# ArchDD/CPP-Raytracer-Rasterizer

Hardware: AMD Instinct MI355X
Metric: Mrays/s (primary+shadow) (higher is better)
Workload: dtype f32

## Files before the change

cpp-raytracer-rasterizer_amd/capi/binned.cpp:

```cpp
#include "capi.hpp"

namespace mirt {


int PairList::ensure(size_t cap)
{
    int r;
    if ((r = dev_realloc(&d_entries, cap)) || (r = dev_realloc(&d_pair_keys, cap)) || (r = dev_realloc(&d_pair_vals, cap)) ||
        (r = dev_realloc(&d_sorted_keys, cap)) || (r = dev_realloc(&d_tmp_vals, cap))) { cap_entries = 0; return r; }
    cap_entries = (uint32_t)cap;
    return MIRT_OK;
}


void PairList::poll()
{
    if (count_pending && hipEventQuery(ev_count) == hipSuccess) {
        known_pairs = *h_count; have_known = true; count_pending = false;
    }
    (void)hipGetLastError();
}

int PairList::record_count()
{
// ... 211 lines not shown
int transient_light_pass(LightPass &L, const float *origins, int nlights, int cube_bins, int tshells, uint32_t per_light, uint64_t lkey, bool *kept,
                         unsigned long long *zero_hits )
{
    int rc;
    const uint64_t key = Fnv(g.scene_version).mix(&lkey, 8).mix(&cube_bins, 4).mix(&tshells, 4).mix(&g.n, 4).mix(&nlights, 4).h;
    const PassPlan plan = L.kept.plan_for(key, nlights, L.pairs);
    *kept = plan.reuse;
    if (plan.reuse) return MIRT_OK;
    if ((rc = ensure_face_lists(L, nlights))) return rc;
    if (nlights > L.light_tab_lights || L.light_tab_n != g.n) {
        if ((rc = dev_grow(&L.d_light_tab, &L.light_tab_lights, nlights, (size_t)nlights * g.n, true))) return rc;
        L.light_tab_n = g.n;
    }
    const uint32_t nkeys = per_light * (uint32_t)nlights;
    if (nkeys + 1 > L.cap_bins && (rc = dev_grow(&L.d_bin_off, &L.cap_bins, nkeys + 1, (size_t)nkeys + 1, true))) return rc;
    if (!L.d_frames) HIP_TRY(hipMalloc(reinterpret_cast<void **>(&L.d_frames), sizeof(BinFrameDesc) * (6 * MIRT_MAX_LIGHTS) + sizeof(float) * 3 * (1 + MIRT_MAX_LIGHTS)));
    struct { BinFrameDesc frames[6 * MIRT_MAX_LIGHTS]; float origins[3 * (1 + MIRT_MAX_LIGHTS)]; } up;
    static_assert(sizeof(BinFrameDesc) % 4 == 0, "descriptors are uploaded as words");
    fill_light_frames(up.frames, origins, nlights, cube_bins, tshells, 0u, g.bbox_lo, g.bbox_hi);
    float *d_origins = reinterpret_cast<float *>(L.d_frames + 6 * nlights);
    memcpy(reinterpret_cast<char *>(up.frames + 6 * nlights), origins, sizeof(float) * 3 * (1 + nlights));
    const ZeroJob zj = { L.d_bin_counters, (int)(LIGHT_COUNTER_BYTES / 4), reinterpret_cast<uint32_t *>(zero_hits), zero_hits ? 2 * HIT_SHARDS * HIT_SHARD_STRIDE : 0 };
    HIP_TRY(upload_small(L.d_frames, &up, sizeof(BinFrameDesc) * 6 * nlights + sizeof(float) * 3 * (1 + nlights), g.stream, &zj));
    if ((rc = cube_bin_chain(L, L.d_frames, d_origins, nlights, nkeys, L.d_light_tab, L.d_bin_off, L.d_bin_counters, &L.kept.bin_entries, plan.may_guess))) return rc;
    L.kept.keep(key, nlights);
    if (L.cap_light_rows < L.pairs.cap_entries && (rc = dev_grow(&L.d_light_rows, &L.cap_light_rows, L.pairs.cap_entries, (size_t)L.pairs.cap_entries, true))) return rc;
    const uint32_t expect = std::max<uint32_t>(L.kept.bin_entries, 1u);
    hipLaunchKernelGGL(k_expand_light_rows, dim3((unsigned)std::min<uint32_t>((expect + 255) / 256, 4096u)), dim3(256), 0, g.stream,
                       L.d_bin_off, L.pairs.d_entries, nlights, per_light, L.d_light_tab, g.n, L.d_light_rows, L.d_bin_counters, L.pairs.cap_used, (uint32_t *)nullptr);
    return MIRT_OK;
}


int OriginTables::ensure_cam_rows() { return cam_tab_n == g.n ? MIRT_OK : dev_grow(&d_cam_tab, &cam_tab_n, g.n, (size_t)g.n, false); }

int BinPass::ensure_counters(size_t bytes)
{
    if (!d_bin_counters) { HIP_TRY(hipMalloc(reinterpret_cast<void **>(&d_bin_counters), bytes)); HIP_TRY(hipMemsetAsync(d_bin_counters, 0, bytes, g.stream)); }
    return MIRT_OK;
}

int CameraPass::ensure_sel()
{
    if (sel_n == g.n) return MIRT_OK;
    kept.forget();
    return dev_grow(&d_sel, &sel_n, g.n, (size_t)g.n, true);
}

SelectOut CameraPass::select_out(const OriginTables &T, int count_word) const
{
    SelectOut so;
    memset(&so, 0, sizeof so);
    so.cam_tab = T.d_cam_tab; so.sel = d_sel;
    so.sel_count = d_bin_counters + count_word; so.sel_count_next = d_bin_counters + (count_word ^ 1);
    return so;
}

static void launch_prep_select(const BinFrameDesc &frame, const SelectOut &so)
{
    const unsigned sel_grid = (unsigned)std::min<long long>(((long long)g.n + 1023) / 1024, (long long)g.cu_count);
    if (sel_grid) hipLaunchKernelGGL(k_prep_select, dim3(sel_grid), dim3(1024), 0, g.stream, g.d_tris, g.n, frame, so);
}

int binned_pass(const mirt_view *view, StreamState &ss, const float *origins, int nlights, int y0, int y1, BinnedPass *bp)
{
    int rc;
    CameraPass &S = ss.cam;
// ... 46 lines not shown
    if (!S.d_frames) HIP_TRY(hipMalloc(reinterpret_cast<void **>(&S.d_frames), sizeof(BinFrameDesc) * (1 + 6 * MIRT_MAX_LIGHTS)));
    const PassPlan plan = S.kept.plan_for(key, bin_mode, S.pairs);
    const uint32_t pairs_x = (uint32_t)((bs.frame0.nbu + 1) / 2);
    uint32_t group_rows[ORDER_GROUPS] = { 0 };
    for (int j = bs.frame0.j0; j < bs.frame0.j1; j++) group_rows[((uint32_t)j >> ORDER_STRIPE_SHIFT) & (ORDER_GROUPS - 1)]++;
    const uint32_t order_seg = pairs_x * *std::max_element(group_rows, group_rows + ORDER_GROUPS);
    const uint32_t *cam_off = S.d_bin_off - (size_t)key_shift_tiles * (size_t)bs.frame0.nshell;
    bool lights_kept = false, forked = false;
    if (transient) {
        static const bool side_off = env_int("MIRT_LIGHT_SIDE_STREAM", 1) == 0;
        hipStream_t main_stream = g.stream;
        forked = !plan.reuse && !side_off;
        if (forked) {
            HIP_TRY(hipEventRecord(ss.ev_fork, main_stream));
            HIP_TRY(hipStreamWaitEvent(ss.aux, ss.ev_fork, 0));
            g.stream = ss.aux;
        }
        rc = transient_light_pass(L, origins, nlights, cube_bins, tshells, per_light, lkey, &lights_kept, plan.reuse ? g.d_hits : nullptr);
        g.stream = main_stream;
        if (rc) return rc;
        if (forked) HIP_TRY(hipEventRecord(ss.ev_join, ss.aux));
    }
    if (plan.reuse) {
        if (!(transient && !lights_kept)) HIP_TRY(hipMemsetAsync(g.d_hits, 0, HIT_BYTES, g.stream));
        g.stats.bins_reused = 1;
    } else {
        S.sel_parity ^= 1;
        SelectOut so = S.select_out(ss.tabs, SEL_COUNT0 + S.sel_parity);
        so.zero_hits = g.d_hits; so.zero_counter = S.d_bin_counters;
        if ((rc = hist_prepare(ss.hist, bs.frame0, &so))) return rc;
        launch_prep_select(bs.frame0, so);
        if ((rc = hist_publish(ss.hist))) return rc;
        bs.sel = S.d_sel; bs.sel_count = so.sel_count;
        g.stats_sel_count = so.sel_count;
        if ((rc = bin_pass(S.pairs, bs, ss.tabs.d_cam_tab, nullptr, S.d_bin_counters, S.d_bin_off, &S.kept.bin_entries, plan.may_guess))) return rc;
        S.kept.keep(key, bin_mode);
        if (order_seg > S.cap_order && (rc = dev_grow(&S.d_order, &S.cap_order, order_seg, (size_t)ORDER_GROUPS * ORDER_CLASSES * order_seg, true))) return rc;
        hipLaunchKernelGGL(k_tile_order, dim3((pairs_x + 63) / 64, (unsigned)(bs.frame0.j1 - bs.frame0.j0)), dim3(64), 0, g.stream, cam_off, bs.frame0.nshell,
                           bs.frame0.nbu, bs.frame0.j0, bs.frame0.j1, S.d_bin_counters, S.pairs.cap_used, S.d_order, order_seg);
    }
    if (forked) HIP_TRY(hipStreamWaitEvent(g.stream, ss.ev_join, 0));
    k_end(MIRT_K_BIN);

    bp->cam_off = cam_off;
    bp->tiles_x = bs.frame0.nbu;
    bp->cam_shells = bs.frame0.nshell;
    bp->shell_d0 = bs.frame0.shell_d0; bp->shell_iw = bs.frame0.shell_iw;
    bp->order_seg = order_seg;
    bp->cube = transient ? cube_view(L, cube_bins, tshells) : cube_view(g.lc);
    bp->light_tab = transient ? L.d_light_tab : g.lc.d_light_tab;
    bp->light_pair_count = transient ? L.d_bin_counters : S.d_bin_counters;
    bp->light_pair_cap = transient ? L.pairs.cap_used : 0xFFFFFFFFu;
    return MIRT_OK;
}

int hist_only_pass(const mirt_view *view)
{
    int rc;
    g.stream = g.cur().stream;
    StreamState &ss = g.cur();
    CameraPass &S = ss.cam;
    if ((rc = ss.tabs.ensure_cam_rows()) || (rc = S.ensure_sel()) || (rc = S.ensure_counters(512))) return rc;
    S.kept.forget();
    const BinFrameDesc fr = make_camera_frame(view, 0, 0, g.aa);
    SelectOut so = S.select_out(ss.tabs, HIST_SEL_COUNT);
    if ((rc = hist_prepare(ss.hist, fr, &so))) return rc;
// ... 62 lines not shown
```

cpp-raytracer-rasterizer_amd/capi/capi.hpp:

```cpp
#pragma once

#include "../csrc/bin_sort.hpp"
#include "../csrc/comm.hpp"
#include "../csrc/cull.hpp"
#include "../csrc/dof.hpp"
#include "../csrc/rt_common.hpp"
#include "../csrc/raster_common.hpp"
#include "../csrc/rt_binned.hpp"
#include "../csrc/rt_trace_frame.hpp"
#include "../csrc/scan.hpp"
#include "../query/rt_query.hpp"
#include "../along/along.hpp"
#include "../along/alongs.hpp"
#include "../grid/ray_grid.hpp"
#include "../order/ordered_hits.hpp"
#include "../lights/many_lights.hpp"
#include "../lights/aa_many_lights.hpp"
#include "cube_plan.hpp"
#include "pass_plan.hpp"
#include "along_plan.hpp"
#include "object_plan.hpp"
#include "dof_plan.hpp"
#include "aa_plan.hpp"
#include "env.hpp"
// ... 30 lines not shown
MIRT_KERNEL void k_tile_order(const uint32_t *, int, int, int, int, uint32_t *, uint32_t, TilePairRec *, uint32_t);
MIRT_KERNEL void k_geo_table(const float *, int, GeoRow *, ShadeRow *);
MIRT_KERNEL void k_expand_light_rows(const uint32_t *, const uint32_t *, int, uint32_t, const OriginRow *, int, LightRow *, const uint32_t *, uint32_t, uint32_t *);
MIRT_KERNEL void k_cull(const float *, int, const CullParams, uint8_t *);
size_t rt_trace_lds_bytes(int waves);
int launch_raster(RasterFrame &f, RasterScratch &s, uint64_t scene_version, hipStream_t stream, hipEvent_t *ev, bool *ev_used);

extern char g_err[512];
int fail(int code, const char *fmt, ...);

#define HIP_TRY(expr)                                                                          \
    do {                                                                                       \
        hipError_t e_ = (expr);                                                                \
        if (e_ != hipSuccess)                                                                  \
            return fail(MIRT_ERR_HIP, "%s failed: %s (%s:%d)", #expr, hipGetErrorString(e_), __FILE__, __LINE__); \
    } while (0)

enum { EV_CALL0 = 0, EV_CALL1 = 1, EV_K0 = 2, EV_COUNT = 2 + 2 * 8 };
constexpr int MAX_FLIGHT = 4;
constexpr int SEL_COUNT0 = 80;
constexpr int HIST_SEL_COUNT = 82;
constexpr int HIST_RING = 4;
constexpr int HIST_SLOTS = HIST_RING + 1;
constexpr size_t HIT_BYTES = sizeof(unsigned long long) * HIT_SHARDS * HIT_SHARD_STRIDE;

struct OriginTables {
    OriginRow *d_cam_tab = nullptr;
    OriginRow *d_light_tab = nullptr;
    int cam_tab_n = 0, light_tab_n = 0, light_tab_lights = 0;
    float *d_origins = nullptr;
    uint32_t *d_flags = nullptr;

    int ensure_cam_rows();
    void release();
};

struct PairList {
    uint32_t *d_entries = nullptr;
    uint32_t *d_pair_keys = nullptr, *d_pair_vals = nullptr, *d_sorted_keys = nullptr;
    uint32_t *d_tmp_vals = nullptr;
    uint32_t *d_bucket = nullptr;
    uint32_t cap_buckets = 0;
    bool bucket_dirty = false;
    uint32_t cap_entries = 0;
    uint32_t cap_used = 0;
    uint32_t *h_count = nullptr;
    hipEvent_t ev_count = nullptr;
    bool count_pending = false;
    bool count_event_due = false;
    bool have_known = false;
    uint32_t known_pairs = 0;

    int ensure(size_t cap);
    void poll();
    int record_count();
    void forget_scene() { have_known = false; count_pending = false; }
    void release();
};

struct KeptPass {
    uint64_t bin_key = 0;
    bool bin_key_valid = false;
    int last_bin_mode = -1;
    uint32_t bin_entries = 0;

    PassPlan plan_for(uint64_t key, int mode, PairList &P) const;
// ... 595 lines not shown
```

cpp-raytracer-rasterizer_amd/csrc/rt_binned.hip:

```cpp
#include "rt_binned.hpp"

#include <float.h>

namespace mirt {

constexpr int BIN_L0 = BIN_COARSE * BIN_COARSE;

struct BinItem {
    float A0[4], A1[4], A2[4], Bu[4], Bv[4];
    float lou, hiu, lov, hiv;
};

__device__ __forceinline__ float bcastf(float v, int lane) { return __builtin_bit_cast(float, __builtin_amdgcn_readlane(__builtin_bit_cast(int, v), lane)); }

__device__ __forceinline__ float corner(float s, float lo, float hi) { return fmaxf(s * lo, s * hi); }

__device__ __forceinline__ bool cell_may_hit(const BinItem &u, const float (&A)[4], float I, float J, float K)
{
    bool ok = true;
#pragma unroll
    for (int k = 0; k < 4; k++) ok = ok && (__builtin_fmaf(J, u.Bv[k], __builtin_fmaf(I, u.Bu[k], A[k])) >= 0.0f);
    return ok && (I + K >= u.lou) && (I <= u.hiu) && (J + K >= u.lov) && (J <= u.hiv);
}

// ... 325 lines not shown
        if (from_cam_list) { chunk = w; frame = 0; list = bs.sel; nhere = nsel; }
        else if (faces_listed) {
            const uint32_t w2 = (uint32_t)(w - ncam);
            int lo = 0, hi = nrest;
            while (hi - lo > 1) { const int mid = (lo + hi) >> 1; if (s_first[mid] <= w2) lo = mid; else hi = mid; }
            chunk = (int)(w2 - s_first[lo]);
            frame = lo + (listed ? 1 : 0);
            list = bs.face_lists + (size_t)lo * bs.face_stride;
            nhere = min(bs.face_counts[lo], (uint32_t)n);
        } else { const int w2 = w - ncam; chunk = w2 / nrest; frame = w2 - chunk * nrest + (listed ? 1 : 0); }
        const int item_tris = from_cam_list ? cam_chunk : chunk_tris;
        const uint32_t slot = (uint32_t)chunk * (uint32_t)item_tris + threadIdx.x;
        const uint32_t tri = ((int)threadIdx.x < item_tris && slot < nhere) ? (list ? list[slot] : slot) : 0xFFFFFFFFu;
        const BinFrameDesc fr = bs.frames ? bs.frames[frame] : bs.frame0;
        BinFrameGrid gr;
        gr.nbu = fr.nbu; gr.fj0 = fr.j0; gr.fj1 = fr.j1; gr.fbase = fr.base; gr.nshell = (uint32_t)max(fr.nshell, 1);
        gr.cells_x = (gr.nbu + BIN_L0 - 1) / BIN_L0; gr.cy0 = gr.fj0 / BIN_L0;
        gr.ncell = gr.cells_x * ((gr.fj1 + BIN_L0 - 1) / BIN_L0 - gr.cy0);
        const int nbu = gr.nbu, fj0 = gr.fj0, fj1 = gr.fj1;
        BinItem it;
        memset(&it, 0, sizeof it);
        int kind = 0;
#ifdef MIRT_BIN_STATS
        int dbg_state = 0;
        bool dbg_joint = false;
#endif
        int i_lo = 0, i_hi = -1, j_lo = 0, j_hi = -1;
        unsigned long long cells = 0;
        uint32_t shell = 0;
        if (tri < (uint32_t)n && fj1 > fj0) {
            const OriginRow &row = (fr.tab == 0) ? cam_tab[tri] : light_tab[(size_t)(fr.tab - 1) * n + tri];
            shell = bin_shell_of(row.r1.w, fr.shell_d0, fr.shell_iw, fr.nshell);
            TriBinFns t = make_bin_fns(row, fr);
            add_bbox(t, tris15 + (size_t)15 * tri, fr);
#ifdef MIRT_BIN_STATS
            dbg_state = t.bstate == BOX_VALID ? 0 : (t.bstate == BOX_NONE ? 1 : 2);
#endif
            const float T = 1.6940658945086007e-21f;
            const bool both = fabsf(t.nb) < T || !(t.nb == t.nb);
            const float sgn = t.nb < 0.0f ? -1.0f : 1.0f;
            const EdgeFn *fn[4] = { &t.n, &t.p, &t.q, &t.s };
            const float inf = __builtin_huge_valf();
#pragma unroll
            for (int k = 0; k < 4; k++) {
                const float su = sgn * fn[k]->cu, sv = sgn * fn[k]->cv;
                const float base = sgn * fn[k]->c0 + fn[k]->m + su * fr.ulo + sv * fr.vlo;
                it.Bu[k] = both ? 0.0f : su * fr.du;
                it.Bv[k] = both ? 0.0f : sv * fr.dv;
                it.A0[k] = both ? inf : base + corner(su, fr.pad_lo, (float)BIN_L0 * fr.du + fr.pad_hi) + corner(sv, fr.pad_lo, (float)BIN_L0 * fr.dv + fr.pad_hi);
                it.A1[k] = both ? inf : base + corner(su, fr.pad_lo, (float)BIN_COARSE * fr.du + fr.pad_hi) + corner(sv, fr.pad_lo, (float)BIN_COARSE * fr.dv + fr.pad_hi);
                it.A2[k] = both ? inf : base + corner(su, fr.pad_lo, fr.du + fr.pad_hi) + corner(sv, fr.pad_lo, fr.dv + fr.pad_hi);
            }
            if (t.bstate == BOX_VALID) {
                box_to_bins(t.bu0, t.bu1, fr.ulo, fr.pad_lo, fr.pad_hi, bin_rcp(fr.du), &it.lou, &it.hiu);
                box_to_bins(t.bv0, t.bv1, fr.vlo, fr.pad_lo, fr.pad_hi, bin_rcp(fr.dv), &it.lov, &it.hiv);
            } else if (t.bstate == BOX_EMPTY) {
                it.lou = it.lov = inf; it.hiu = it.hiv = -inf;
            } else {
                it.lou = it.lov = -inf; it.hiu = it.hiv = inf;
            }
            const float flo_u = fmaxf(ceilf(it.lou) - 1.0f, 0.0f), fhi_u = fminf(floorf(it.hiu), (float)(nbu - 1));
            const float flo_v = fmaxf(ceilf(it.lov) - 1.0f, (float)fj0), fhi_v = fminf(floorf(it.hiv), (float)(fj1 - 1));
            if (flo_u <= fhi_u && flo_v <= fhi_v) {
                i_lo = (int)flo_u; i_hi = (int)fhi_u; j_lo = (int)flo_v; j_hi = (int)fhi_v;
                kind = (i_hi - i_lo < BIN_DIRECT_SIDE && j_hi - j_lo < BIN_DIRECT_SIDE) ? 1 : 2;
            }
// ... 163 lines not shown
```

cpp-raytracer-rasterizer_amd/csrc/rt_binned.hpp:

```cpp
#pragma once

#include "rt_common.hpp"

namespace mirt {

#ifndef MIRT_ORDER_STRIPE_SHIFT
#define MIRT_ORDER_STRIPE_SHIFT 2
#endif
constexpr int ORDER_STRIPE_SHIFT = MIRT_ORDER_STRIPE_SHIFT;
constexpr int BIN_TILE = 8;
constexpr int BIN_COARSE = 8;
constexpr int CUBE_BINS_MIN = 64;
constexpr int MAX_BIN_FRAMES = 1 + 6 * MIRT_MAX_LIGHTS;

struct BinFrameDesc {
    float P0[3], Pu[3], Pv[3];
    float S[3];
    float ru[3], rv[3], rw[3];
    float ulo, vlo, du, dv;
    float pad_lo, pad_hi;
    float dmax;
    int nbu, nbv;
    int j0, j1;
    uint32_t base;
// ... 6 lines not shown
{
    if (nshell <= 1) return 0u;
    const float s = (near - d0) * iw;
#ifdef __HIP_DEVICE_COMPILE__
    return (uint32_t)min(max((int)s, 0), nshell - 1);
#else
    if (!(s >= 0.0f)) return 0u;
    return s >= (float)(nshell - 1) ? (uint32_t)(nshell - 1) : (uint32_t)(int)s;
#endif
}

struct GeoRow { float4 g0, g1, g2; };
struct ShadeRow { float4 n, col; };
typedef OriginRow LightRow;

struct BinSet {
    const BinFrameDesc *frames;
    BinFrameDesc frame0;
    int nframes;
    uint32_t nbins;
    uint32_t *bin_off;
    uint32_t *entries;
    uint32_t cap_entries;
    uint32_t *counters;
    uint32_t *bucket_cnt;
    uint32_t nbuckets;
    int bucket_shift;
    int chunk_tris;
    const uint32_t *sel;
    const uint32_t *sel_count;
    const uint32_t *face_lists;
    const uint32_t *face_counts;
    uint32_t face_stride;
};

constexpr int SEL_HIST_MAX = 256;
struct SelectOut {
    OriginRow *cam_tab;
    uint32_t *sel;
    uint32_t *sel_count;
    uint32_t *sel_count_next;
    uint32_t *hist;
    int hist_shift;
    uint32_t *zero_faces;
    int zero_faces_n;
    unsigned long long *zero_hits;
    uint32_t *zero_counter;
};

struct BinPairs {
    uint32_t *keys;
    uint32_t *vals;
    uint32_t cap;
};

struct EdgeFn { float c0, cu, cv, m; };

MIRT_HD EdgeFn make_edge_fn(float gx, float gy, float gz, const BinFrameDesc &fr)
{
    EdgeFn e;
    e.c0 = gx * fr.P0[0] + gy * fr.P0[1] + gz * fr.P0[2];
    e.cu = gx * fr.Pu[0] + gy * fr.Pu[1] + gz * fr.Pu[2];
    e.cv = gx * fr.Pv[0] + gy * fr.Pv[1] + gz * fr.Pv[2];
    e.m = 7.62939453125e-06f * ((fabsf(gx) + fabsf(gy) + fabsf(gz)) * fr.dmax) + 9.5367431640625e-07f;
    return e;
}

struct TriBinFns {
    EdgeFn n, p, q, s;
    float nb;
    float bu0, bu1, bv0, bv1;
    int bstate;
};
enum { BOX_NONE = 0, BOX_VALID = 1, BOX_EMPTY = 2 };

MIRT_HD TriBinFns make_bin_fns(const OriginRow &r, const BinFrameDesc &fr)
{
    TriBinFns t;
    t.n = make_edge_fn(r.r0.x, r.r0.y, r.r0.z, fr);
    t.p = make_edge_fn(r.r1.x, r.r1.y, r.r1.z, fr);
    t.q = make_edge_fn(r.r2.x, r.r2.y, r.r2.z, fr);
    t.s.c0 = t.n.c0 - t.p.c0 - t.q.c0;
    t.s.cu = t.n.cu - t.p.cu - t.q.cu;
    t.s.cv = t.n.cv - t.p.cv - t.q.cv;
    t.s.m = 1.25f * (t.n.m + t.p.m + t.q.m);
    t.nb = r.r0.w;
    t.bu0 = t.bu1 = t.bv0 = t.bv1 = 0.0f;
    t.bstate = BOX_NONE;
    return t;
}

#ifdef __HIP_DEVICE_COMPILE__
MIRT_HD float bin_rcp(float x) { return __builtin_amdgcn_rcpf(x); }
MIRT_HD float bin_rsq(float x) { return __builtin_amdgcn_rsqf(x); }
#else
#ifndef MIRT_BIN_HOST_RCP
#define MIRT_BIN_HOST_RCP(x) (1.0f / (x))
#define MIRT_BIN_HOST_RSQ(x) (1.0f / sqrtf(x))
#endif
MIRT_HD float bin_rcp(float x) { return MIRT_BIN_HOST_RCP(x); }
MIRT_HD float bin_rsq(float x) { return MIRT_BIN_HOST_RSQ(x); }
#endif

MIRT_HD void add_bbox(TriBinFns &t, const float *t15, const BinFrameDesc &fr)
{
    const float UP = 1.0000019073486328125f, DOWN = 0.99999809265136719f;
    float us[3], vs[3], pad = 0.0f;
    int front = 0, behind = 0;
#pragma unroll
    for (int j = 0; j < 3; j++) {
        const float gx = fr.S[0] - t15[3 * j], gy = fr.S[1] - t15[3 * j + 1], gz = fr.S[2] - t15[3 * j + 2];
        const float w = fr.rw[0] * gx + fr.rw[1] * gy + fr.rw[2] * gz;
        const float wm = fabsf(fr.rw[0] * gx) + fabsf(fr.rw[1] * gy) + fabsf(fr.rw[2] * gz);
        front += (w > 0.00390625f * wm);
        behind += (w < -0.00390625f * wm);
        const float un = fr.ru[0] * gx + fr.ru[1] * gy + fr.ru[2] * gz, vn = fr.rv[0] * gx + fr.rv[1] * gy + fr.rv[2] * gz;
        const float um = fabsf(fr.ru[0] * gx) + fabsf(fr.ru[1] * gy) + fabsf(fr.ru[2] * gz);
        const float vm = fabsf(fr.rv[0] * gx) + fabsf(fr.rv[1] * gy) + fabsf(fr.rv[2] * gz);
        us[j] = un / w; vs[j] = vn / w;
        const float iw = bin_rcp(fabsf(w));
        pad = fmaxf(pad, 4.76837158203125e-07f * ((um + fabsf(us[j]) * wm) * iw + (vm + fabsf(vs[j]) * wm) * iw) +
                             2.384185791015625e-07f * (fabsf(us[j]) + fabsf(vs[j])));
// ... 154 lines not shown
```

cpp-raytracer-rasterizer_amd/csrc/rt_trace.hip:

```cpp
#include "rt_trace_frame.hpp"

#include <float.h>

namespace mirt {


__global__ __launch_bounds__(256) void k_geo_table(const float *__restrict__ tris15, int n, GeoRow *__restrict__ geo, ShadeRow *__restrict__ shade)
{
    const int t = blockIdx.x * blockDim.x + threadIdx.x;
    if (t >= n) return;
    const float *t15 = tris15 + (size_t)15 * t;
    const v3 v0 = ld3(t15), e1 = sub3(ld3(t15 + 3), v0), e2 = sub3(ld3(t15 + 6), v0);
    GeoRow g;
    g.g0 = make_float4(v0.x, v0.y, v0.z, e1.x);
    g.g1 = make_float4(e1.y, e1.z, e2.x, e2.y);
    g.g2 = make_float4(e2.z, 0.0f, 0.0f, 0.0f);
    geo[t] = g;
    const v3 nd = normalize3(ld3(t15 + 9));
    ShadeRow sr;
    sr.n = make_float4(nd.x, nd.y, nd.z, 0.0f);
    sr.col = make_float4(t15[12], t15[13], t15[14], 0.0f);
    shade[t] = sr;
}

__global__ __launch_bounds__(256) void k_expand_light_rows(const uint32_t *__restrict__ bin_off, const uint32_t *__restrict__ entries,
                                                           int nlights, uint32_t keys_per_light,
                                                           const OriginRow *__restrict__ light_tab, int n,
                                                           LightRow *__restrict__ rows, const uint32_t *__restrict__ pair_count, uint32_t pair_cap,
                                                           uint32_t *__restrict__ row_tri )
{
    if (pair_count && *pair_count > pair_cap) return;
    const uint32_t first = bin_off[0], total = bin_off[(size_t)nlights * keys_per_light];
    for (uint32_t p = first + blockIdx.x * blockDim.x + threadIdx.x; p < total; p += gridDim.x * blockDim.x) {
        int k = 0;
        while (k + 1 < nlights && bin_off[(size_t)(k + 1) * keys_per_light] <= p) k++;
        const uint32_t tri = entries[p];
        rows[p] = light_tab[(size_t)k * n + tri];
        if (row_tri) row_tri[p] = tri;
    }
}

#ifndef MIRT_TR_STAGE
#define MIRT_TR_STAGE 16
#endif
constexpr int TR_STAGE = MIRT_TR_STAGE;
constexpr int TR_DRAIN = 64;
constexpr int TR_QUEUE = 96;
constexpr int TR_PIX = 128;
static_assert(TR_STAGE == 16, "the staging lanes are split 16 / 16 between the two tiles");

struct TrWaveLds {
    union {
        struct {
            float4 rows[TR_STAGE * 6];
            float4 geo[TR_STAGE * 2 * 3];
        };
        struct {
            float4 ray[TR_PIX];
            uint8_t sink;
        };
    };
    float4 q[TR_QUEUE];
    unsigned long long best[TR_PIX];
    uint2 qa[TR_QUEUE];
    union {
        float px[TR_PIX];
        float thr[TR_PIX];
    };
    float py[TR_PIX], pz[TR_PIX];
    uint8_t flag[TR_PIX];
};
static_assert(sizeof(TrWaveLds) % 16 == 0, "per-wave LDS slice must keep 16-byte alignment");
static_assert(sizeof(TrWaveLds) == 8064, "20 waves share a CU's LDS: the ray table overlays the staging, it adds nothing");

__device__ __forceinline__ void wave_lds_fence()
{
    __builtin_amdgcn_fence(__ATOMIC_RELEASE, "wavefront");
    __builtin_amdgcn_wave_barrier();
    __builtin_amdgcn_fence(__ATOMIC_ACQUIRE, "wavefront");
}

template <bool SHADOW>
__device__ __forceinline__ void tr_drain(TrWaveLds &s, int lane, int count, const float4 *__restrict__ geo, v3 start,
                                         const uint32_t *__restrict__ row_tri = nullptr, bool lazy_geo = false)
{
    wave_lds_fence();
    if (lane < count) {
        const float4 e = s.q[lane];
        uint2 a = s.qa[lane];
        float t, u, v;
        div3_sel(e.w, e.y, e.z, e.x, __builtin_amdgcn_ballot_w64(exact_quotients_outside(e.w, e.y, e.z, e.x)), t, u, v);
        if (u + v <= 1.0f && u >= 0.0f && v >= 0.0f && t >= 0.0f) {
            float4 g0, g1, g2;
            if (SHADOW) {
                const uint32_t tri = row_tri ? row_tri[a.y] : a.y;
                const float4 *g = geo + (size_t)tri * 3;
                g0 = g[0]; g1 = g[1]; g2 = g[2];
            } else if (lazy_geo) {
                const float4 *g = geo + (size_t)a.y * 3;
                g0 = g[0]; g1 = g[1]; g2 = g[2];
                a.x &= 0xFFu;
            } else {
                const float4 *g = s.geo + (a.x >> 8) * 3;
                g0 = g[0]; g1 = g[1]; g2 = g[2];
                a.x &= 0xFFu;
            }
            const v3 v0 = V3(g0.x, g0.y, g0.z), e1 = V3(g0.w, g1.x, g1.y), e2 = V3(g1.z, g1.w, g2.x);
            const v3 p = add3(add3(v0, scale3(e1, u)), scale3(e2, v));
            const float dist = distance3(start, p);
            if (SHADOW) {
                if (dist < s.thr[a.x]) s.flag[a.x] = 1;
            } else {
                s.flag[a.x] = 1;
                const unsigned long long key = min_t_key(dist, (int)a.y);
                atomicMin(&s.best[a.x], key);
                __builtin_amdgcn_fence(__ATOMIC_ACQ_REL, "wavefront");
                if (s.best[a.x] == key) { s.px[a.x] = p.x; s.py[a.x] = p.y; s.pz[a.x] = p.z; }
            }
        }
    }
    wave_lds_fence();
}

template <bool SHADOW>
__device__ __forceinline__ void tr_drain_full(TrWaveLds &s, int lane, int &qn, const float4 *__restrict__ geo, v3 start,
                                              const uint32_t *__restrict__ row_tri = nullptr, bool lazy_geo = false)
{
    tr_drain<SHADOW>(s, lane, TR_DRAIN, geo, start, row_tri, lazy_geo);
    const int rest = qn - TR_DRAIN;
    float4 e = make_float4(0.0f, 0.0f, 0.0f, 0.0f);
    uint2 a = make_uint2(0u, 0u);
    if (lane < rest) { e = s.q[TR_DRAIN + lane]; a = s.qa[TR_DRAIN + lane]; }
    wave_lds_fence();
    if (lane < rest) { s.q[lane] = e; s.qa[lane] = a; }
    qn = rest;
    wave_lds_fence();
}

__device__ __forceinline__ unsigned long long wballot(bool p) { return __builtin_amdgcn_ballot_w64(p); }

__device__ __forceinline__ int wave_rank(unsigned long long m)
{
    return (int)__builtin_amdgcn_mbcnt_hi((uint32_t)(m >> 32), __builtin_amdgcn_mbcnt_lo((uint32_t)m, 0u));
}

__device__ __forceinline__ void cube_bin_of2(const v3p &rd, uint32_t face_base0, int cube_bins, uint32_t *bin0, uint32_t *bin1)
{
    f2 a, b, m;
    int face[2];
#pragma unroll
    for (int h = 0; h < 2; h++) {
        const float x = h ? rd.x.y : rd.x.x, y = h ? rd.y.y : rd.y.x, z = h ? rd.z.y : rd.z.x;
        const float ax = fabsf(x), ay = fabsf(y), az = fabsf(z);
        int k;
        float mm, aa, bb, sgn;
        if (ax >= ay && ax >= az) { k = 0; mm = ax; sgn = x; aa = y; bb = z; }
        else if (ay >= az) { k = 1; mm = ay; sgn = y; aa = z; bb = x; }
        else { k = 2; mm = az; sgn = z; aa = x; bb = y; }
        face[h] = 2 * k + (sgn < 0.0f ? 1 : 0);
        if (h) { a.y = aa; b.y = bb; m.y = mm; } else { a.x = aa; b.x = bb; m.x = mm; }
    }
// ... 99 lines not shown
            sum += cnt[c];
            const bool past = w >= sum;
            first = past ? sum : first;
            cls = past ? c - 1 : cls;
        }
        if (cls < 0) return;
        const uint32_t at = w - first;
        const uint4 r4 = *reinterpret_cast<const uint4 *>(tf.order + ((size_t)group * ORDER_CLASSES + (uint32_t)cls) * tf.order_seg + at);
        rec.txy = r4.x; rec.beg = r4.y; rec.nA = r4.z; rec.nB = r4.w;
    }
    const int txA = (int)(rec.txy & 0xFFFFu), ty = (int)(rec.txy >> 16);
    const bool enB = txA + 1 < tf.tiles_x;
    const int xA = txA * BIN_TILE + (lane & 7), xB = xA + BIN_TILE, y = ty * BIN_TILE + (lane >> 3);
    const bool okY = y >= f.y0 && y < f.y1;
    const bool okA = okY && xA < W, okB = enB && okY && xB < W;
    const unsigned long long okmA = wballot(okA), okmB = wballot(okB);
    const unsigned nokA = (unsigned)__popcll(okmA), nokB = (unsigned)__popcll(okmB);
#ifdef MIRT_TR_TIMING
    const long long tm0 = __builtin_amdgcn_s_memtime();
    long long tm_last = tm0, tm_seg[10] = { 0, 0, 0, 0, 0, 0, 0, 0, 0, 0 };
#define TM_SEG(i) { const long long now_ = __builtin_amdgcn_s_memtime(); tm_seg[i] += now_ - tm_last; tm_last = now_; }
#else
#define TM_SEG(i)
#endif
    const bool brute = npairs > tf.pair_cap;
    const bool brute_l = nlpairs > tf.light_pair_cap;
    const v3 cam = ld3(f.cam);
    const int rs = AA ? f.aa : 1;

    const uint32_t begA = rec.beg, begB = rec.beg + rec.nA;
    const uint32_t nall = brute ? min(nsel, (uint32_t)f.n) : 0u;
    const uint32_t nA = brute ? nall : rec.nA, nB = brute ? (enB ? nall : 0u) : rec.nB;
    const float4 *geo4 = reinterpret_cast<const float4 *>(tf.geo);
    const bool lazy = (flags & TRF_LAZY_GEO) != 0u;
    const bool list_end = (flags & TRF_LIST_END) != 0u && !brute;
    TM_SEG(0)

    float bdA = FLT_MAX, bdB = FLT_MAX;
    int biA = -1, biB = -1;
    v3 posA = V3(0.0f, 0.0f, 0.0f), posB = posA;
    v3p avg = splat3(V3(0.0f, 0.0f, 0.0f));
    unsigned ntests = 0, ncand = 0, nsteps_p = 0, nsteps_s = 0, ndrains = 0;
    unsigned ncand_l = 0;
    int qn = 0;
    const float hw = (float)W / 2.0f, hh = (float)H / 2.0f;

    f2 y1 = splat2(aa_start(y, rs));
    for (int z = 0; z < rs; z++) {
        f2 x1 = { aa_start(xA, rs), aa_start(xB, rs) };
        for (int z2 = 0; z2 < rs; z2++) {
            const v3p d = V3P(x1 - splat2(hw), y1 - splat2(hh), splat2(f.focal));
            const v3p nd = neg3p(mat3_mul_vecp(f.rot, d));

            s.best[lane] = MIN_T_NONE; s.best[lane + 64] = MIN_T_NONE;
            s.flag[lane] = 0; s.flag[lane + 64] = 0;
            float lbA = okA ? FLT_MAX : -__builtin_huge_valf(), lbB = okB ? FLT_MAX : -__builtin_huge_valf();
            float tbA = FLT_MAX, tbB = FLT_MAX;
            uint32_t liveA = nA, liveB = nB;
            for (uint32_t base = 0; base < max(liveA, liveB); base += TR_STAGE) {
                const int cntA = (int)min((uint32_t)TR_STAGE, liveA > base ? liveA - base : 0u);
                const int cntB = (int)min((uint32_t)TR_STAGE, liveB > base ? liveB - base : 0u);
                if (STATS) ncand += nokA * (unsigned)cntA + nokB * (unsigned)cntB;
                wave_lds_fence();
                float my_near = 0.0f;
                const int sh = lane >> 4, sj = lane & 15;
                const bool stage = lane < 32 && sj < (sh ? cntB : cntA);
                if (stage) {
                    const uint32_t idx = brute ? tf.sel[base + (uint32_t)sj] : tf.cam_entries[(sh ? begB : begA) + base + (uint32_t)sj];
                    const float4 *src = reinterpret_cast<const float4 *>(f.cam_tab + idx);
                    const float4 a0 = src[0], a1 = src[1], a2 = src[2];
                    if (!lazy) {
                        const float4 *gsrc = geo4 + (size_t)idx * 3;
                        float4 *gdst = s.geo + lane * 3;
                        gdst[0] = gsrc[0]; gdst[1] = gsrc[1]; gdst[2] = gsrc[2];
                    }
                    float *dst = reinterpret_cast<float *>(s.rows) + sj * 24 + sh;
                    dst[0] = a0.x; dst[2] = a0.y; dst[4] = a0.z; dst[6] = a0.w;
                    dst[8] = a1.x; dst[10] = a1.y; dst[12] = a1.z; dst[14] = a1.w;
                    dst[16] = a2.x; dst[18] = a2.y; dst[20] = a2.z; dst[22] = __uint_as_float(idx);
                    my_near = a1.w;
                } else if (lane < 32) {
                    reinterpret_cast<float *>(s.rows)[sj * 24 + sh + 14] = __builtin_huge_valf();
                }
                wave_lds_fence();
                TM_SEG(1)
                uint32_t pmA = (uint32_t)wballot(stage && sh == 0 && !(my_near > tbA)) & 0xFFFFu;
                uint32_t pmB = (uint32_t)(wballot(stage && sh == 1 && !(my_near > tbB)) >> 16) & 0xFFFFu;
                uint32_t pm = pmA | pmB;
                while (pm) {
                    const int j = __builtin_ctz(pm);
                    pm &= pm - 1u;
                    if (STATS) nsteps_p++;
                    const float4 *R = s.rows + 6 * j;
                    const float4 R0 = R[0], R1 = R[1], R2 = R[2], R3 = R[3], R4 = R[4], R5 = R[5];
                    TestDots2 td;
                    td.den = (f2){ R0.x, R0.y } * nd.x + (f2){ R0.z, R0.w } * nd.y + (f2){ R1.x, R1.y } * nd.z;
                    td.pu = (f2){ R2.x, R2.y } * nd.x + (f2){ R2.z, R2.w } * nd.y + (f2){ R3.x, R3.y } * nd.z;
                    td.qv = (f2){ R4.x, R4.y } * nd.x + (f2){ R4.z, R4.w } * nd.y + (f2){ R5.x, R5.y } * nd.z;
                    const f2 fm = maybe_hit2_margin(td);
                    const unsigned long long nearA = wballot(!(R3.z > lbA)), nearB = wballot(!(R3.w > lbB));
                    const unsigned long long filtA = wballot(fm.x >= MAYBE_HIT_THRESHOLD), filtB = wballot(fm.y >= MAYBE_HIT_THRESHOLD);
                    const unsigned long long mA = nearA & filtA, mB = nearB & filtB;
                    const bool passA0 = (mA >> lane) & 1ull, passB = (mB >> lane) & 1ull;
                    if (STATS) ntests += (unsigned)__popcll(nearA) + (unsigned)__popcll(nearB);
                    if (mA | mB) {
                        int cA = __popcll(mA);
                        const int cB = __popcll(mB);
                        bool passA = passA0;
                        if (qn + cA + cB > TR_QUEUE) {
                            TM_SEG(2)
                            if (qn) { tr_drain<false>(s, lane, qn, geo4, cam, nullptr, lazy); qn = 0; if (STATS) ndrains++; }
                            if (cA + cB > TR_QUEUE) {
                                if (passA) {
                                    const int at = wave_rank(mA);
                                    s.q[at] = make_float4(td.den.x, td.pu.x, td.qv.x, R1.z);
                                    s.qa[at] = make_uint2((uint32_t)lane | ((uint32_t)j << 8), __float_as_uint(R5.z));
                                }
                                tr_drain<false>(s, lane, cA, geo4, cam, nullptr, lazy); if (STATS) ndrains++;
                                passA = false; cA = 0;
                            }
                            TM_SEG(3)
                        }
                        if (passA) {
                            const int at = qn + wave_rank(mA);
                            s.q[at] = make_float4(td.den.x, td.pu.x, td.qv.x, R1.z);
                            s.qa[at] = make_uint2((uint32_t)lane | ((uint32_t)j << 8), __float_as_uint(R5.z));
                        }
                        if (passB) {
                            const int at = qn + cA + wave_rank(mB);
                            s.q[at] = make_float4(td.den.y, td.pu.y, td.qv.y, R1.w);
                            s.qa[at] = make_uint2(((uint32_t)lane + 64u) | ((uint32_t)(16 + j) << 8), __float_as_uint(R5.w));
                        }
                        qn += cA + cB;
                        if (qn >= TR_DRAIN) {
                            TM_SEG(2)
                            do { tr_drain_full<false>(s, lane, qn, geo4, cam, nullptr, lazy); if (STATS) ndrains++; } while (qn >= TR_DRAIN);
                            TM_SEG(3)
                            lbA = okA ? min_t_dist(s.best[lane]) : lbA; lbB = okB ? min_t_dist(s.best[lane + 64]) : lbB;
                            tbA = wave_max_f(lbA); tbB = wave_max_f(lbB);
                            pmA &= (uint32_t)wballot(stage && sh == 0 && !(my_near > tbA));
                            pmB &= (uint32_t)(wballot(stage && sh == 1 && !(my_near > tbB)) >> 16);
                            pm &= pmA | pmB;
                        }
                    }
                }
                TM_SEG(2)
                const bool more = base + TR_STAGE < max(liveA, liveB);
                if (qn) {
                    tr_drain<false>(s, lane, qn, geo4, cam, nullptr, lazy); qn = 0; if (STATS) ndrains++;
                    if (more) {
                        lbA = okA ? min_t_dist(s.best[lane]) : lbA; lbB = okB ? min_t_dist(s.best[lane + 64]) : lbB;
                        tbA = wave_max_f(lbA); tbB = wave_max_f(lbB);
                    }
                }
                if (more && list_end) {
                    const bool later = stage && bin_shell_of(my_near, tf.shell_d0, tf.shell_iw, tf.cam_shells) >
                                                bin_shell_of(sh ? tbB : tbA, tf.shell_d0, tf.shell_iw, tf.cam_shells);
                    const uint32_t lm = (uint32_t)wballot(later);
                    if (lm & 0xFFFFu) liveA = min(liveA, base + (uint32_t)TR_STAGE);
                    if (lm >> 16) liveB = min(liveB, base + (uint32_t)TR_STAGE);
                }
                TM_SEG(3)
            }
            const unsigned long long keyA = s.best[lane], keyB = s.best[lane + 64];
            const bool anyA = s.flag[lane] != 0, anyB = s.flag[lane + 64] != 0;
            if constexpr (AA) {
                if (anyA && bdA >= min_t_dist(keyA)) {
                    bdA = min_t_dist(keyA); biA = min_t_index(keyA);
                    posA = V3(s.px[lane], s.py[lane], s.pz[lane]);
                }
                if (anyB && bdB >= min_t_dist(keyB)) {
                    bdB = min_t_dist(keyB); biB = min_t_index(keyB);
                    posB = V3(s.px[lane + 64], s.py[lane + 64], s.pz[lane + 64]);
                }
            } else {
                const v3 hpA = V3(s.px[lane], s.py[lane], s.pz[lane]);
                const v3 hpB = V3(s.px[lane + 64], s.py[lane + 64], s.pz[lane + 64]);
                const bool takeA = anyA && bdA >= min_t_dist(keyA), takeB = anyB && bdB >= min_t_dist(keyB);
                bdA = takeA ? min_t_dist(keyA) : bdA; biA = takeA ? min_t_index(keyA) : biA;
                posA = V3(takeA ? hpA.x : posA.x, takeA ? hpA.y : posA.y, takeA ? hpA.z : posA.z);
                bdB = takeB ? min_t_dist(keyB) : bdB; biB = takeB ? min_t_index(keyB) : biB;
                posB = V3(takeB ? hpB.x : posB.x, takeB ? hpB.y : posB.y, takeB ? hpB.z : posB.z);
// ... 214 lines not shown
```

Measured before the change: 57140.

## Precompute per-triangle screen-space filter rows and defer exact test to drain

The binning kernel now writes a per-triangle filter row (three edge functions linear in screen x/y plus the near distance) beside the camera origin table, which is grown to twice its size to hold them. The primary trace stages these compact 5-float4 rows instead of 6-float4 origin rows and filters candidates with three FMAs per edge rather than dot products with the ray direction. The exact den/pu/qv dots are moved into the drain step, computed from geometry and origin data staged per candidate in LDS. This trades less per-pixel filter arithmetic and LDS traffic for more global loads per staged triangle and extra work in the drain, and removes the lazy-geometry path.

```diff
diff --git a/cpp-raytracer-rasterizer_amd/capi/binned.cpp b/cpp-raytracer-rasterizer_amd/capi/binned.cpp
--- a/cpp-raytracer-rasterizer_amd/capi/binned.cpp
+++ b/cpp-raytracer-rasterizer_amd/capi/binned.cpp
@@ -267,7 +267,7 @@
 }
 
 
-int OriginTables::ensure_cam_rows() { return cam_tab_n == g.n ? MIRT_OK : dev_grow(&d_cam_tab, &cam_tab_n, g.n, (size_t)g.n, false); }
+int OriginTables::ensure_cam_rows() { return cam_tab_n == g.n ? MIRT_OK : dev_grow(&d_cam_tab, &cam_tab_n, g.n, (size_t)2 * g.n, false); }
 
 int BinPass::ensure_counters(size_t bytes)
 {
@@ -380,6 +380,7 @@
         launch_prep_select(bs.frame0, so);
         if ((rc = hist_publish(ss.hist))) return rc;
         bs.sel = S.d_sel; bs.sel_count = so.sel_count;
+        bs.cam_filt = ss.tabs.cam_filt();
         g.stats_sel_count = so.sel_count;
         if ((rc = bin_pass(S.pairs, bs, ss.tabs.d_cam_tab, nullptr, S.d_bin_counters, S.d_bin_off, &S.kept.bin_entries, plan.may_guess))) return rc;
         S.kept.keep(key, bin_mode);
diff --git a/cpp-raytracer-rasterizer_amd/capi/capi.hpp b/cpp-raytracer-rasterizer_amd/capi/capi.hpp
--- a/cpp-raytracer-rasterizer_amd/capi/capi.hpp
+++ b/cpp-raytracer-rasterizer_amd/capi/capi.hpp
@@ -86,6 +86,7 @@
     uint32_t *d_flags = nullptr;
 
     int ensure_cam_rows();
+    FilterRow *cam_filt() const { return reinterpret_cast<FilterRow *>(d_cam_tab + cam_tab_n); }
     void release();
 };
 
diff --git a/cpp-raytracer-rasterizer_amd/csrc/rt_binned.hip b/cpp-raytracer-rasterizer_amd/csrc/rt_binned.hip
--- a/cpp-raytracer-rasterizer_amd/csrc/rt_binned.hip
+++ b/cpp-raytracer-rasterizer_amd/csrc/rt_binned.hip
@@ -381,6 +381,7 @@
             const OriginRow &row = (fr.tab == 0) ? cam_tab[tri] : light_tab[(size_t)(fr.tab - 1) * n + tri];
             shell = bin_shell_of(row.r1.w, fr.shell_d0, fr.shell_iw, fr.nshell);
             TriBinFns t = make_bin_fns(row, fr);
+            if (bs.cam_filt && fr.tab == 0) bs.cam_filt[tri] = make_filter_row(t, row.r1.w, tri);
             add_bbox(t, tris15 + (size_t)15 * tri, fr);
 #ifdef MIRT_BIN_STATS
             dbg_state = t.bstate == BOX_VALID ? 0 : (t.bstate == BOX_NONE ? 1 : 2);
diff --git a/cpp-raytracer-rasterizer_amd/csrc/rt_binned.hpp b/cpp-raytracer-rasterizer_amd/csrc/rt_binned.hpp
--- a/cpp-raytracer-rasterizer_amd/csrc/rt_binned.hpp
+++ b/cpp-raytracer-rasterizer_amd/csrc/rt_binned.hpp
@@ -62,6 +62,7 @@
     const uint32_t *face_lists;
     const uint32_t *face_counts;
     uint32_t face_stride;
+    struct FilterRow *cam_filt;
 };
 
 constexpr int SEL_HIST_MAX = 256;
@@ -118,6 +119,37 @@
     t.bu0 = t.bu1 = t.bv0 = t.bv1 = 0.0f;
     t.bstate = BOX_NONE;
     return t;
+}
+
+struct FilterRow { float4 a, b, c; };
+static_assert(sizeof(FilterRow) == 48, "a filter row is three 16-byte loads, like the origin row it stands beside");
+
+MIRT_HD FilterRow make_filter_row(const TriBinFns &t, float near, uint32_t tri)
+{
+    const float T = 1.6940658945086007e-21f;
+    const float sgn = t.nb < 0.0f ? -1.0f : 1.0f;
+    float f[9] = { sgn * t.p.c0 + t.p.m, sgn * t.p.cu, sgn * t.p.cv, sgn * t.q.c0 + t.q.m, sgn * t.q.cu, sgn * t.q.cv,
+                   sgn * t.s.c0 + t.s.m, sgn * t.s.cu, sgn * t.s.cv };
+    float mag = 0.0f;
+#pragma unroll
+    for (int i = 0; i < 9; i++) mag += fabsf(f[i]);
+    if (fabsf(t.nb) < T || !(t.nb == t.nb) || !(mag < 1.0e30f)) {
+#pragma unroll
+        for (int i = 0; i < 9; i++) f[i] = (i % 3 == 0) ? __builtin_huge_valf() : 0.0f;
+    }
+    FilterRow r;
+    r.a = make_float4(f[0], f[1], f[2], f[3]);
+    r.b = make_float4(f[4], f[5], f[6], f[7]);
+    r.c = make_float4(f[8], near, __builtin_bit_cast(float, tri), 0.0f);
+    return r;
+}
+
+MIRT_HD bool filter_row_pass(const FilterRow &r, float x, float y)
+{
+    const float A = __builtin_fmaf(r.a.z, y, __builtin_fmaf(r.a.y, x, r.a.x));
+    const float B = __builtin_fmaf(r.b.y, y, __builtin_fmaf(r.b.x, x, r.a.w));
+    const float S = __builtin_fmaf(r.c.x, y, __builtin_fmaf(r.b.w, x, r.b.z));
+    return !(fminf(fminf(A, B), S) < 0.0f);
 }
 
 #ifdef __HIP_DEVICE_COMPILE__
diff --git a/cpp-raytracer-rasterizer_amd/csrc/rt_trace.hip b/cpp-raytracer-rasterizer_amd/csrc/rt_trace.hip
--- a/cpp-raytracer-rasterizer_amd/csrc/rt_trace.hip
+++ b/cpp-raytracer-rasterizer_amd/csrc/rt_trace.hip
@@ -49,11 +49,14 @@
 constexpr int TR_PIX = 128;
 static_assert(TR_STAGE == 16, "the staging lanes are split 16 / 16 between the two tiles");
 
+constexpr int TR_FROW = 5;
+struct TrCand { float2 w[7]; };
+static_assert(sizeof(TrCand) == 56, "32 staged candidates take the place the 32 geometry rows had");
 struct TrWaveLds {
     union {
         struct {
-            float4 rows[TR_STAGE * 6];
-            float4 geo[TR_STAGE * 2 * 3];
+            float4 rows[TR_STAGE * TR_FROW];
+            TrCand cand[TR_STAGE * 2];
         };
         struct {
             float4 ray[TR_PIX];
@@ -82,30 +85,33 @@
 
 template <bool SHADOW>
 __device__ __forceinline__ void tr_drain(TrWaveLds &s, int lane, int count, const float4 *__restrict__ geo, v3 start,
-                                         const uint32_t *__restrict__ row_tri = nullptr, bool lazy_geo = false)
+                                         const uint32_t *__restrict__ row_tri = nullptr)
 {
     wave_lds_fence();
     if (lane < count) {
-        const float4 e = s.q[lane];
+        float4 e = s.q[lane];
         uint2 a = s.qa[lane];
+        v3 v0 = V3(0.0f, 0.0f, 0.0f), e1 = v0, e2 = v0;
+        if (!SHADOW) {
+            const TrCand &c = s.cand[a.x >> 8];
+            const float2 c0 = c.w[0], c1 = c.w[1], c2 = c.w[2], c3 = c.w[3], c4 = c.w[4], c5 = c.w[5], c6 = c.w[6];
+            v0 = V3(c0.x, c0.y, c1.x); e1 = V3(c1.y, c2.x, c2.y); e2 = V3(c3.x, c3.y, c4.x);
+            const v3 b = sub3(start, v0), be2 = cross3(b, e2), e1b = cross3(e1, b);
+            const TestDots td = test_dots(make_float4(c4.y, c5.x, c5.y, c6.x), make_float4(be2.x, be2.y, be2.z, 0.0f),
+                                          make_float4(e1b.x, e1b.y, e1b.z, 0.0f), V3(e.x, e.y, e.z));
+            e = make_float4(td.den, td.pu, td.qv, c6.x);
+            a.y = __float_as_uint(c6.y);
+            a.x &= 0xFFu;
+        }
         float t, u, v;
         div3_sel(e.w, e.y, e.z, e.x, __builtin_amdgcn_ballot_w64(exact_quotients_outside(e.w, e.y, e.z, e.x)), t, u, v);
         if (u + v <= 1.0f && u >= 0.0f && v >= 0.0f && t >= 0.0f) {
-            float4 g0, g1, g2;
             if (SHADOW) {
                 const uint32_t tri = row_tri ? row_tri[a.y] : a.y;
                 const float4 *g = geo + (size_t)tri * 3;
-                g0 = g[0]; g1 = g[1]; g2 = g[2];
-            } else if (lazy_geo) {
-                const float4 *g = geo + (size_t)a.y * 3;
-                g0 = g[0]; g1 = g[1]; g2 = g[2];
-                a.x &= 0xFFu;
-            } else {
-                const float4 *g = s.geo + (a.x >> 8) * 3;
-                g0 = g[0]; g1 = g[1]; g2 = g[2];
-                a.x &= 0xFFu;
-            }
-            const v3 v0 = V3(g0.x, g0.y, g0.z), e1 = V3(g0.w, g1.x, g1.y), e2 = V3(g1.z, g1.w, g2.x);
+                const float4 g0 = g[0], g1 = g[1], g2 = g[2];
+                v0 = V3(g0.x, g0.y, g0.z); e1 = V3(g0.w, g1.x, g1.y); e2 = V3(g1.z, g1.w, g2.x);
+            }
             const v3 p = add3(add3(v0, scale3(e1, u)), scale3(e2, v));
             const float dist = distance3(start, p);
             if (SHADOW) {
@@ -124,9 +130,9 @@
 
 template <bool SHADOW>
 __device__ __forceinline__ void tr_drain_full(TrWaveLds &s, int lane, int &qn, const float4 *__restrict__ geo, v3 start,
-                                              const uint32_t *__restrict__ row_tri = nullptr, bool lazy_geo = false)
-{
-    tr_drain<SHADOW>(s, lane, TR_DRAIN, geo, start, row_tri, lazy_geo);
+                                              const uint32_t *__restrict__ row_tri = nullptr)
+{
+    tr_drain<SHADOW>(s, lane, TR_DRAIN, geo, start, row_tri);
     const int rest = qn - TR_DRAIN;
     float4 e = make_float4(0.0f, 0.0f, 0.0f, 0.0f);
     uint2 a = make_uint2(0u, 0u);
@@ -292,7 +298,7 @@
     const uint32_t nall = brute ? min(nsel, (uint32_t)f.n) : 0u;
     const uint32_t nA = brute ? nall : rec.nA, nB = brute ? (enB ? nall : 0u) : rec.nB;
     const float4 *geo4 = reinterpret_cast<const float4 *>(tf.geo);
-    const bool lazy = (flags & TRF_LAZY_GEO) != 0u;
+    const FilterRow *filt = reinterpret_cast<const FilterRow *>(f.cam_tab + f.n);
     const bool list_end = (flags & TRF_LIST_END) != 0u && !brute;
     TM_SEG(0)
 
@@ -328,19 +334,22 @@
                 if (stage) {
                     const uint32_t idx = brute ? tf.sel[base + (uint32_t)sj] : tf.cam_entries[(sh ? begB : begA) + base + (uint32_t)sj];
                     const float4 *src = reinterpret_cast<const float4 *>(f.cam_tab + idx);
-                    const float4 a0 = src[0], a1 = src[1], a2 = src[2];
-                    if (!lazy) {
-                        const float4 *gsrc = geo4 + (size_t)idx * 3;
-                        float4 *gdst = s.geo + lane * 3;
-                        gdst[0] = gsrc[0]; gdst[1] = gsrc[1]; gdst[2] = gsrc[2];
-                    }
-                    float *dst = reinterpret_cast<float *>(s.rows) + sj * 24 + sh;
-                    dst[0] = a0.x; dst[2] = a0.y; dst[4] = a0.z; dst[6] = a0.w;
-                    dst[8] = a1.x; dst[10] = a1.y; dst[12] = a1.z; dst[14] = a1.w;
-                    dst[16] = a2.x; dst[18] = a2.y; dst[20] = a2.z; dst[22] = __uint_as_float(idx);
-                    my_near = a1.w;
+                    const float4 *fsrc = reinterpret_cast<const float4 *>(filt + idx);
+                    const float4 *gsrc = geo4 + (size_t)idx * 3;
+                    const float4 a0 = src[0];
+                    const float4 g0 = gsrc[0], g1 = gsrc[1], g2 = gsrc[2];
+                    const float4 f0 = fsrc[0], f1 = fsrc[1], f2 = fsrc[2];
+                    TrCand &cd = s.cand[lane];
+                    cd.w[0] = make_float2(g0.x, g0.y); cd.w[1] = make_float2(g0.z, g0.w); cd.w[2] = make_float2(g1.x, g1.y);
+                    cd.w[3] = make_float2(g1.z, g1.w); cd.w[4] = make_float2(g2.x, a0.x); cd.w[5] = make_float2(a0.y, a0.z);
+                    cd.w[6] = make_float2(a0.w, __uint_as_float(idx));
+                    float *dst = reinterpret_cast<float *>(s.rows) + sj * (4 * TR_FROW) + sh;
+                    dst[0] = f0.x; dst[2] = f0.y; dst[4] = f0.z; dst[6] = f0.w;
+                    dst[8] = f1.x; dst[10] = f1.y; dst[12] = f1.z; dst[14] = f1.w;
+                    dst[16] = f2.x; dst[18] = f2.y;
+                    my_near = f2.y;
                 } else if (lane < 32) {
-                    reinterpret_cast<float *>(s.rows)[sj * 24 + sh + 14] = __builtin_huge_valf();
+                    reinterpret_cast<float *>(s.rows)[sj * (4 * TR_FROW) + sh + 18] = __builtin_huge_valf();
                 }
                 wave_lds_fence();
                 TM_SEG(1)
@@ -351,15 +360,14 @@
                     const int j = __builtin_ctz(pm);
                     pm &= pm - 1u;
                     if (STATS) nsteps_p++;
-                    const float4 *R = s.rows + 6 * j;
-                    const float4 R0 = R[0], R1 = R[1], R2 = R[2], R3 = R[3], R4 = R[4], R5 = R[5];
-                    TestDots2 td;
-                    td.den = (f2){ R0.x, R0.y } * nd.x + (f2){ R0.z, R0.w } * nd.y + (f2){ R1.x, R1.y } * nd.z;
-                    td.pu = (f2){ R2.x, R2.y } * nd.x + (f2){ R2.z, R2.w } * nd.y + (f2){ R3.x, R3.y } * nd.z;
-                    td.qv = (f2){ R4.x, R4.y } * nd.x + (f2){ R4.z, R4.w } * nd.y + (f2){ R5.x, R5.y } * nd.z;
-                    const f2 fm = maybe_hit2_margin(td);
-                    const unsigned long long nearA = wballot(!(R3.z > lbA)), nearB = wballot(!(R3.w > lbB));
-                    const unsigned long long filtA = wballot(fm.x >= MAYBE_HIT_THRESHOLD), filtB = wballot(fm.y >= MAYBE_HIT_THRESHOLD);
+                    const float4 *R = s.rows + TR_FROW * j;
+                    const float4 R0 = R[0], R1 = R[1], R2 = R[2], R3 = R[3], R4 = R[4];
+                    const f2 fa = __builtin_elementwise_fma((f2){ R1.x, R1.y }, y1, __builtin_elementwise_fma((f2){ R0.z, R0.w }, x1, (f2){ R0.x, R0.y }));
+                    const f2 fb = __builtin_elementwise_fma((f2){ R2.z, R2.w }, y1, __builtin_elementwise_fma((f2){ R2.x, R2.y }, x1, (f2){ R1.z, R1.w }));
+                    const f2 fs = __builtin_elementwise_fma((f2){ R4.x, R4.y }, y1, __builtin_elementwise_fma((f2){ R3.z, R3.w }, x1, (f2){ R3.x, R3.y }));
+                    const float fmA = fminf(fminf(fa.x, fb.x), fs.x), fmB = fminf(fminf(fa.y, fb.y), fs.y);
+                    const unsigned long long nearA = wballot(!(R4.z > lbA)), nearB = wballot(!(R4.w > lbB));
+                    const unsigned long long filtA = wballot(!(fmA < 0.0f)), filtB = wballot(!(fmB < 0.0f));
                     const unsigned long long mA = nearA & filtA, mB = nearB & filtB;
                     const bool passA0 = (mA >> lane) & 1ull, passB = (mB >> lane) & 1ull;
                     if (STATS) ntests += (unsigned)__popcll(nearA) + (unsigned)__popcll(nearB);
@@ -369,32 +377,32 @@
                         bool passA = passA0;
                         if (qn + cA + cB > TR_QUEUE) {
                             TM_SEG(2)
-                            if (qn) { tr_drain<false>(s, lane, qn, geo4, cam, nullptr, lazy); qn = 0; if (STATS) ndrains++; }
+                            if (qn) { tr_drain<false>(s, lane, qn, geo4, cam); qn = 0; if (STATS) ndrains++; }
                             if (cA + cB > TR_QUEUE) {
                                 if (passA) {
                                     const int at = wave_rank(mA);
-                                    s.q[at] = make_float4(td.den.x, td.pu.x, td.qv.x, R1.z);
-                                    s.qa[at] = make_uint2((uint32_t)lane | ((uint32_t)j << 8), __float_as_uint(R5.z));
+                                    s.q[at] = make_float4(nd.x.x, nd.y.x, nd.z.x, 0.0f);
+                                    s.qa[at] = make_uint2((uint32_t)lane | ((uint32_t)j << 8), 0u);
                                 }
-                                tr_drain<false>(s, lane, cA, geo4, cam, nullptr, lazy); if (STATS) ndrains++;
+                                tr_drain<false>(s, lane, cA, geo4, cam); if (STATS) ndrains++;
                                 passA = false; cA = 0;
                             }
                             TM_SEG(3)
                         }
                         if (passA) {
                             const int at = qn + wave_rank(mA);
-                            s.q[at] = make_float4(td.den.x, td.pu.x, td.qv.x, R1.z);
-                            s.qa[at] = make_uint2((uint32_t)lane | ((uint32_t)j << 8), __float_as_uint(R5.z));
+                            s.q[at] = make_float4(nd.x.x, nd.y.x, nd.z.x, 0.0f);
+                            s.qa[at] = make_uint2((uint32_t)lane | ((uint32_t)j << 8), 0u);
                         }
                         if (passB) {
                             const int at = qn + cA + wave_rank(mB);
-                            s.q[at] = make_float4(td.den.y, td.pu.y, td.qv.y, R1.w);
-                            s.qa[at] = make_uint2(((uint32_t)lane + 64u) | ((uint32_t)(16 + j) << 8), __float_as_uint(R5.w));
+                            s.q[at] = make_float4(nd.x.y, nd.y.y, nd.z.y, 0.0f);
+                            s.qa[at] = make_uint2(((uint32_t)lane + 64u) | ((uint32_t)(16 + j) << 8), 0u);
                         }
                         qn += cA + cB;
                         if (qn >= TR_DRAIN) {
                             TM_SEG(2)
-                            do { tr_drain_full<false>(s, lane, qn, geo4, cam, nullptr, lazy); if (STATS) ndrains++; } while (qn >= TR_DRAIN);
+                            do { tr_drain_full<false>(s, lane, qn, geo4, cam); if (STATS) ndrains++; } while (qn >= TR_DRAIN);
                             TM_SEG(3)
                             lbA = okA ? min_t_dist(s.best[lane]) : lbA; lbB = okB ? min_t_dist(s.best[lane + 64]) : lbB;
                             tbA = wave_max_f(lbA); tbB = wave_max_f(lbB);
@@ -407,7 +415,7 @@
                 TM_SEG(2)
                 const bool more = base + TR_STAGE < max(liveA, liveB);
                 if (qn) {
-                    tr_drain<false>(s, lane, qn, geo4, cam, nullptr, lazy); qn = 0; if (STATS) ndrains++;
+                    tr_drain<false>(s, lane, qn, geo4, cam); qn = 0; if (STATS) ndrains++;
                     if (more) {
                         lbA = okA ? min_t_dist(s.best[lane]) : lbA; lbB = okB ? min_t_dist(s.best[lane + 64]) : lbB;
                         tbA = wave_max_f(lbA); tbB = wave_max_f(lbB);
```

Result: no change. 57160, median of 2 (+0.0%).
